# AdeeshKolluru/AdsorbDiff

Hardware: AMD Instinct MI355X
Metric: sampled adsorbate sites/sec (50 denoise steps, ~200-atom slabs) (higher is better)
Workload: dtype f32 (f16x3-split MFMA, fp32 accumulate; ADF_GEMM=f32 selects exact f32)

## Files before the change

adsorbdiff_amd/csrc/api.hip:

```cpp
#include <stdarg.h>
#include <stdlib.h>
#include <string.h>

#include <new>

#include "common.h"

static thread_local char g_err[512] = "";

void adf_set_error(const char* fmt, ...) {
    va_list ap;
    va_start(ap, fmt);
    vsnprintf(g_err, sizeof(g_err), fmt, ap);
    va_end(ap);
}

extern "C" const char* adf_last_error(void) { return g_err; }
extern "C" const char* adf_version(void) { return "adsorbdiff_hip 0.5.0 (gfx950)"; }

adf_tune adf_tune_from_env() {
    auto off_is_0 = [](const char* name) { const char* e = getenv(name); return (e && atoi(e) == 0) ? 0 : 1; };
    auto is_f32 = [](const char* name) { const char* e = getenv(name); return e && strcmp(e, "f32") == 0; };
    adf_tune t = {};
    t.gemm_stream = off_is_0("ADF_GEMM_STREAM");
    t.head_gate_fused = off_is_0("ADF_HEAD_GATE_FUSED");
    t.lift_emit = off_is_0("ADF_LIFT_EMIT");
    t.graph_sys_csr = off_is_0("ADF_GRAPH_SYS_CSR");
    t.train_gemm16 = is_f32("ADF_TRAIN_GEMM") ? 0 : 1;
    t.wgrad_f32 = is_f32("ADF_WGRAD") ? 1 : 0;
    const char* gt = getenv("ADF_EQV2_GEMM_TILE");
    t.eqv2_gemm_tile256 = (gt && atoi(gt) == 128) ? 0 : 1;
    t.eqv2_rotin_generic = getenv("ADF_EQV2_ROTIN_GENERIC") != nullptr;
    t.eqv2_rotout_generic = getenv("ADF_EQV2_ROTOUT_GENERIC") != nullptr;
    return t;
}
const adf_tune& adf_tune_process() {
    static const adf_tune t = adf_tune_from_env();
    return t;
}
int adf_current_num_cus() {
    int dev = 0, n = 0;
    if (hipGetDevice(&dev) != hipSuccess || hipDeviceGetAttribute(&n, hipDeviceAttributeMultiprocessorCount, dev) != hipSuccess) return 0;
    return n;
}

extern "C" int32_t adf_profile_enable(adf_painn_t h, int32_t on) {
    if (!h) { adf_set_error("null handle"); return ADF_EINVAL; }
    h->prof.enable(on != 0);
    ADF_HIP_CHECK(hipMemset(h->kcount, 0, 8 * sizeof(unsigned long long)));
    return ADF_OK;
}

extern "C" int32_t adf_profile_read(adf_painn_t h, float* ms, int64_t* count, int64_t* message_ksteps, void* stream) {
    if (!h || !ms || !count) { adf_set_error("null argument"); return ADF_EINVAL; }
    ADF_HIP_CHECK(hipStreamSynchronize((hipStream_t)stream));
    if (message_ksteps) {
        unsigned long long k[8];
        ADF_HIP_CHECK(hipMemcpy(k, h->kcount, sizeof(k), hipMemcpyDeviceToHost));
        ADF_HIP_CHECK(hipMemset(h->kcount, 0, sizeof(k)));
        *message_ksteps = (int64_t)k[0];
    }
    return h->prof.read(ms, count, ADF_PROF_NCAT);
// ... 347 lines not shown
    ADF_HIP_CHECK(hipMemcpyAsync(&e, h->nptr + N, sizeof(int32_t), hipMemcpyDeviceToHost, s));
    ADF_HIP_CHECK(hipStreamSynchronize(s));
    if (num_edges) *num_edges = e;
    return ADF_OK;
}

static int32_t zero_pad_rows(adf_painn* h, int N, hipStream_t s) {
    const size_t row = (size_t)5 * h->hp.hidden_channels;
    ADF_HIP_CHECK(hipMemsetAsync(h->rec + (size_t)N * row, 0, sizeof(float) * row, s));
    return ADF_OK;
}

static int32_t make_records(adf_painn* h, int l, int n, const float* x, const float* vec, bool vec_is_zero, float* rec,
                            const int32_t* row_map, hipStream_t s) {
    const int H = h->hp.hidden_channels;
    const adf_layer_weights& w = h->layer[l];
    if (n <= 0) return ADF_OK;
    adf_prof_begin(h, ADF_PROF_NODE, s);
    const bool lift = h->lift_on && !h->gemm_f32;
    const bool em = lift && h->tune.lift_emit;
    ADF_TRY(adf_nodewise_layernorm(x, w.ln_w, w.ln_b, h->y, n, H, s, em ? h->mag_a : nullptr, h->rows_dev));
    ADF_TRY(adf_linear(h, h->y, H, w.xp0_w, &w.xp0_16, w.xp0_b, h->cat, H, n, H, H, 1, s, em ? h->mag_a : nullptr,
                       em ? h->mag_b : nullptr));
    if (h->gemm_f32) {
        if (row_map) { adf_set_error("internal: mapped records need the f16x3 path"); return ADF_EINVAL; }
        ADF_TRY(adf_launch_gemm(h->cat, H, w.xp2_w, H, w.xp2_b, h->xh, 3 * H, n, 3 * H, H, 0, s));
        ADF_TRY(adf_pack_records(h, n, h->xh, vec, vec_is_zero, s, rec));
    } else {
        adf_epi ep = {};
        ep.vec_in = vec; ep.rec = rec ? rec : h->rec; ep.H = H; ep.vec_is_zero = vec_is_zero ? 1 : 0;
        ep.row_map = row_map;
        ep.rmag = em ? h->mag_b : nullptr;
        ep.m_dev = h->rows_dev;
        ADF_TRY(adf_launch_gemm16_fused(h->cat, H, &w.xp2_16, n, H, H, 1, &ep, s, h->tune, lift ? &h->lift : nullptr));
    }
    adf_prof_end(h, s);
    return ADF_OK;
}

static int32_t message_layer(adf_painn* h, int l, int N, const float* x, const float* vec, float* x_out,
                             float* vec_out, bool vec_is_zero, hipStream_t s, const int32_t* tlist = nullptr,
                             int n_targets = 0, float* rec = nullptr, bool records_ready = false) {
    if (!records_ready) ADF_TRY(make_records(h, l, N, x, vec, vec_is_zero, rec, nullptr, s));
    adf_prof_begin(h, ADF_PROF_MESSAGE, s);
    const int items = tlist ? n_targets : N;
    const bool emit = h->rmx && h->lift_on && !h->gemm_f32 && !h->msg_f32 && items > 0 && items <= h->part_stride;
    h->part_x = h->part_vec = nullptr;
    const int32_t st = adf_message_impl(h, l, N, x, h->xh, vec, x_out, vec_out, vec_is_zero, s, tlist, n_targets, rec,
                                        tlist ? h->rows_dev : nullptr, emit ? h->xpart : nullptr, h->vpart, h->part_stride);
    if (st == ADF_OK && emit) {
        h->part_x = x_out; h->part_vec = vec_out; h->part_n = items; h->part_dev = tlist ? h->rows_dev : nullptr;
        h->dbg_msg_rows = items;
    }
    adf_prof_end(h, s);
    return st;
}

static int32_t update_layer(adf_painn* h, int l, int N, float* x, float* vec, hipStream_t s, bool from_message = true) {
    const int H = h->hp.hidden_channels;
    const adf_layer_weights& w = h->layer[l];
    adf_prof_begin(h, ADF_PROF_NODE, s);
    const bool parts = from_message && h->rmx && h->lift_on && !h->gemm_f32 && N > 0 && h->part_x == x && h->part_vec == vec &&
                       h->part_n == N && h->part_dev == h->rows_dev;
    h->part_x = h->part_vec = nullptr;
    if (h->gemm_f32) {
        ADF_TRY(adf_launch_gemm(vec, H, w.vp_w, H, nullptr, h->vv, 2 * H, 3 * N, 2 * H, H, 0, s));
        ADF_TRY(adf_nodewise_update_prep(h->vv, x, h->cat, h->dot, N, H, s));
// ... 3 lines not shown
        ep.v1 = h->vv; ep.dotw = h->dot; ep.cat = h->cat; ep.H = H; ep.m_dev = h->rows_dev;
        const adf_lift* lf = h->lift_on ? &h->lift : nullptr;
        if (parts) {
            ADF_TRY(adf_launch_rowmax_combine(h->vpart, 3 * h->part_stride, H / ADF_SLICE_CH, 3ll * N, h->lift.buf, s, h->rows_dev, 3));
            ep.rmag = h->lift.buf;
            if (h->dbg_capture) ADF_HIP_CHECK(hipMemcpyAsync(h->dbg_mag, h->lift.buf, sizeof(float) * 3 * (size_t)N, hipMemcpyDeviceToDevice, s));
        }
        if (parts || (h->dbg_capture && h->rmx && lf && N <= h->part_stride)) {
            ep.catpart = h->catpart; ep.part_stride = h->part_stride; h->dbg_cat_rows = N;
        }
        ADF_TRY(adf_launch_gemm16_fused(vec, H, &w.vp_16, N, H, H, 3, &ep, s, h->tune, lf));
        if (parts) {
            ADF_TRY(adf_launch_rowmax_combine(h->xpart, h->part_stride, H / ADF_SLICE_CH + H / 32, N, h->lift.buf, s, h->rows_dev, 1));
            if (h->dbg_capture) {
                ADF_HIP_CHECK(hipMemcpyAsync(h->dbg_mag + 3 * h->part_stride, h->lift.buf, sizeof(float) * (size_t)N, hipMemcpyDeviceToDevice, s));
                h->dbg_comb_rows = N;
            }
        }
        adf_epi e0 = {};
        e0.A2 = h->cat; e0.K1 = H; e0.m_dev = h->rows_dev;
        e0.rmag = parts ? h->lift.buf : nullptr;
        e0.out_mag = h->lift_on ? reinterpret_cast<unsigned int*>(h->mag_b) : nullptr;
        ADF_TRY(adf_launch_gemm16(x, H, &w.xv0_16, w.xv0_b, h->y, H, N, H, 2 * H, 1, &e0, s, lf, h->tune, h->num_cus));
    }
    int32_t st;
    if (h->gemm_f32) {
        ADF_TRY(adf_launch_gemm(h->y, H, w.xv2_w, H, w.xv2_b, h->xh, 3 * H, N, 3 * H, H, 0, s));
        st = adf_nodewise_update_apply(h->xh, h->dot, h->vv, x, vec, h->scale[l], N, H, s);
    } else {
        adf_epi ep = {};
        ep.x = x; ep.vec = vec; ep.dot = h->dot; ep.vv = h->vv; ep.scale = h->scale[l]; ep.H = H;
        ep.rmag = h->lift_on ? h->mag_b : nullptr;
        ep.m_dev = h->rows_dev;
        st = adf_launch_gemm16_fused(h->y, H, &w.xv2_16, N, H, H, 2, &ep, s, h->tune);
    }
    adf_prof_end(h, s);
    return st;
}

extern "C" int32_t adf_painn_message_layer(adf_painn_t h, int32_t layer, int32_t N, const float* x, const float* vec,
                                           float* x_out, float* vec_out, void* stream) {
    if (!h || !h->weights_set || layer < 0 || layer >= h->hp.num_layers || N != h->lastN) {
        adf_set_error("message_layer: bad handle/layer, or N differs from the built graph");
        return ADF_EINVAL;
    }
    hipStream_t s = (hipStream_t)stream;
    ADF_TRY(zero_pad_rows(h, N, s));
    ADF_TRY(message_layer(h, layer, N, x, vec, x_out, vec_out, false, s));
    return ADF_OK;
}

extern "C" int32_t adf_painn_update_layer(adf_painn_t h, int32_t layer, int32_t N, float* x, float* vec, void* stream) {
    if (!h || !h->weights_set || layer < 0 || layer >= h->hp.num_layers) {
        adf_set_error("update_layer: bad handle/layer");
        return ADF_EINVAL;
    }
    ADF_TRY(ensure_capacity(h, N, 1));
    return update_layer(h, layer, N, x, vec, (hipStream_t)stream, false);
}

extern "C" int32_t adf_painn_get_tune(adf_painn_t h, adf_tune* out) {
    if (!h || !out) { adf_set_error("get_tune: null handle or output"); return ADF_EINVAL; }
    *out = h->tune;
    return ADF_OK;
}

extern "C" int32_t adf_painn_debug_row_maxima(adf_painn_t h, int32_t which, float* out, int64_t capacity, int32_t* rows,
// ... 527 lines not shown
```

adsorbdiff_amd/csrc/common.h:

```cpp
#pragma once
#include <hip/hip_runtime.h>
#include <stdint.h>
#include <stdio.h>
#include <string>
#include <vector>

#include "../../include/adsorbdiff_hip.h"

#define ADF_GROUP_NODES 32
#define ADF_SLICE_CH 64
#define ADF_MAX_CAND 1024
#define ADF_MAX_K 128
#define ADF_NFLAGS 8
#define ADF_MAX_INDEG 1024
#define ADF_MAX_LAYERS 16

void adf_set_error(const char* fmt, ...);

#define ADF_HIP_CHECK(expr)                                                             \
    do {                                                                                \
        hipError_t _e = (expr);                                                         \
        if (_e != hipSuccess) {                                                         \
            adf_set_error("%s failed: %s (%s:%d)", #expr, hipGetErrorString(_e),        \
                          __FILE__, __LINE__);                                          \
// ... 243 lines not shown
    int32_t last_reps[3];
    int num_cus;
    adf_prof prof;
    unsigned long long* kcount;
    adf_pool m_life;
    adf_pool m_ws;
    adf_pool m_inc;
    adf_pool m_sub;
    adf_pool m_rec0;
};

enum { ADF_PROF_GRAPH = 0, ADF_PROF_MESSAGE = 1, ADF_PROF_NODE = 2, ADF_PROF_HEADS = 3, ADF_PROF_STEPPER = 4 };
static inline void adf_prof_begin(adf_painn* h, int cat, hipStream_t s) { h->prof.begin(cat, s); }
static inline void adf_prof_end(adf_painn* h, hipStream_t s) { h->prof.end(s); }

int32_t adf_launch_gemm(const float* A, int lda, const float* W, int ldw, const float* bias, float* C, int ldc,
                        int M, int N, int K, int act_ssilu, hipStream_t s);
adf_tune adf_tune_from_env();
const adf_tune& adf_tune_process();
int adf_current_num_cus();
int32_t adf_launch_gemm16(const float* A, int lda, const adf_w16* W, const float* bias, float* C, int ldc, int M,
                          int N, int K, int act_ssilu, const adf_epi* ep, hipStream_t s, const adf_lift* lf,
                          const adf_tune& tune, int num_cus);
int32_t adf_launch_rowmag(const float* A, int lda, int K1, const float* A2, int K2, long long M, float* mag, hipStream_t s,
                          const int32_t* m_dev = nullptr, int m_mul = 1);
int32_t adf_launch_rowmax_combine(const float* part, long long stride, int nparts, long long M, float* mag, hipStream_t s,
                                  const int32_t* m_dev = nullptr, int m_mul = 1);
int32_t adf_split_weight(const float* w, long long n, adf_w16* out, unsigned int* scratch_bits, hipStream_t s,
                         int perm_H = 0, int K = 0, const float* bias = nullptr, int parts = 3);
int32_t adf_launch_gemm16_vecnorm(const float* A, int lda, const adf_w16* W, float* nrm, int M, int N, int K,
                                  hipStream_t s, const adf_tune& tune, const adf_lift* lf = nullptr,
                                  const float* premag = nullptr);
int32_t adf_launch_gemm16_fused(const float* A, int lda, const adf_w16* W, int M, int H, int K, int epi,
                                const adf_epi* ep, hipStream_t s, const adf_tune& tune, const adf_lift* lf = nullptr);
static inline int32_t adf_linear(const adf_painn* h, const float* A, int lda, const float* W, const adf_w16* W16,
                                 const float* bias, float* C, int ldc, int M, int N, int K, int act, hipStream_t s,
                                 const float* premag = nullptr, float* out_mag = nullptr) {
    if (h->gemm_f32) return adf_launch_gemm(A, lda, W, K, bias, C, ldc, M, N, K, act, s);
    adf_epi ep = {};
    ep.m_dev = h->rows_dev;
    if (h->lift_on) { ep.rmag = premag; ep.out_mag = reinterpret_cast<unsigned int*>(out_mag); }
    return adf_launch_gemm16(A, lda, W16, bias, C, ldc, M, N, K, act, &ep, s, h->lift_on ? &h->lift : nullptr, h->tune,
                             h->num_cus);
}
int32_t adf_pack_frag(const adf_w16* w, int N, int K, void* out, hipStream_t s);
int32_t adf_graph_build_impl(adf_painn* h, const adf_batch* b, hipStream_t s);
int32_t adf_energy_sum(const float* y, int H2, const float* w, const float* bias, const int32_t* atom_offset, float* energy,
                       int num_systems, hipStream_t s);
__device__ __forceinline__ float adf_row16_max(float v) {
#define ADF_ROR(n_) __int_as_float(__builtin_amdgcn_update_dpp(0, __float_as_int(v), 0x120 + (n_), 0xf, 0xf, false))
    v = fmaxf(v, ADF_ROR(8));
    v = fmaxf(v, ADF_ROR(4));
    v = fmaxf(v, ADF_ROR(2));
    v = fmaxf(v, ADF_ROR(1));
#undef ADF_ROR
    return v;
}
__device__ __forceinline__ float adf_half32_max_hi(float v) {
    v = adf_row16_max(v);
    return fmaxf(v, __int_as_float(__builtin_amdgcn_update_dpp(0, __float_as_int(v), 0x142, 0xa, 0xf, false)));
}
__device__ __forceinline__ float adf_lane8_max(float v) {
#define ADF_DPP(c_) __int_as_float(__builtin_amdgcn_update_dpp(0, __float_as_int(v), (c_), 0xf, 0xf, false))
    v = fmaxf(v, ADF_DPP(0xb1));
    v = fmaxf(v, ADF_DPP(0x4e));
    v = fmaxf(v, ADF_DPP(0x141));
#undef ADF_DPP
// ... 77 lines not shown
```

adsorbdiff_amd/csrc/gemm16.hip:

```cpp
#include <stdlib.h>

#include "common.h"

typedef float f32x16 __attribute__((ext_vector_type(16)));
typedef _Float16 half8 __attribute__((ext_vector_type(8)));
typedef _Float16 half4 __attribute__((ext_vector_type(4)));

#ifndef EPI_ABL
#define EPI_ABL 0
#endif
#ifndef G16_ABL
#define G16_ABL 0
#endif
#define HK 32
#define TLD3 96
#define TLD2 64
#define HLD 40

__device__ __forceinline__ float adf_pow2_lift(float mx) {
    if (!(mx > 0.f) || !(mx < 3.0e38f)) return 1.0f;
    int e;
    (void)frexpf(mx, &e);
    e = 15 - e;
    e = e > 120 ? 120 : (e < -120 ? -120 : e);
    return ldexpf(1.0f, e);
}

__device__ __forceinline__ float ssilu16(float x) {
    float s = x / (1.0f + expf(-x));
    return s * 1.6666666666666667f;
}

struct g16_tile {
    int NWN;
    int MI, NJ;
    int NT;
    int TM, TN;
    int ROWS;
};
constexpr g16_tile g16_tile_of(int epi, bool stream) {
    const int nwm = stream ? 1 : 2, nwn = stream ? 4 : 2;
    const int mi = epi >= 3 ? 3 : (epi ? 2 : (stream ? 3 : 2));
    const int nj = epi >= 3 ? 2 : (epi ? 3 : (stream ? 2 : 4));
    const int tm = 32 * mi * nwm;
    return {nwn, mi, nj, 64 * nwm * nwn, tm, 32 * nj * nwn, epi >= 3 ? tm / 3 : tm};
}

template <int ACT, int EPI, bool STREAM>
__global__ __launch_bounds__(g16_tile_of(EPI, STREAM).NT, 2) void adf_gemm_f16x3_kernel(
    const float* __restrict__ A, int lda, const _Float16* __restrict__ Whi, const _Float16* __restrict__ Wlo,
    const float* __restrict__ inv_scale, const float* __restrict__ bias, float* __restrict__ C, int ldc, int Mh, int N,
    int K, int tiles_n, adf_epi ep) {
    constexpr g16_tile geo = g16_tile_of(EPI, STREAM);
    constexpr int MI = geo.MI, NJ = geo.NJ, NWN = geo.NWN, NT = geo.NT, TM = geo.TM, TN = geo.TN;
    const int M = ep.m_dev ? min(Mh, (int)*ep.m_dev) : Mh;
    constexpr int NA = TM * 8 / NT;
    static_assert(TM * 8 % NT == 0, "A staging: whole float4s per thread");
    constexpr int LDS_STREAM = 4 * TM * HLD > NT / 64 * 6400 ? 4 * TM * HLD : NT / 64 * 6400;
    constexpr int LDS_MAIN = STREAM ? LDS_STREAM : (2 * TM + 2 * TN) * HLD;
    constexpr int LDS_REC = EPI == 1 ? NT / 64 * 2048 : 0;
    __shared__ __attribute__((aligned(16))) _Float16 lds[LDS_MAIN + LDS_REC];
    __shared__ float rinv[TM];
    _Float16* Ahi = lds;
    _Float16* Alo = Ahi + TM * HLD;
    _Float16* Bhi = Alo + TM * HLD;
    _Float16* Blo = Bhi + TN * HLD;
    const int tid = threadIdx.x;
    const int lane = tid & 63;
    const int wave = tid >> 6;
    const int wm = (wave / NWN) * (32 * MI);
    const int wn = (wave % NWN) * (32 * NJ);

    const int id = blockIdx.x;
    const int xcd = id & 7;
    const int qd = id >> 3;
    const int tile_m = (qd / tiles_n) * 8 + xcd;
    const int tile_n = qd % tiles_n;
    const int m0 = tile_m * geo.ROWS;
    const int n0 = tile_n * TN;
    if (m0 >= M) return;

    unsigned int a_goff[NA];
    int a_off[NA];
    float a_rs[NA];
    auto global_row = [&](int row) -> unsigned int {
        if constexpr (EPI >= 3) {
            const int atom = m0 + (row / 96) * 32 + (row & 31), ax = (row % 96) >> 5;
            return (unsigned int)min(atom, M - 1) * 3u + ax;
        } else {
            return (unsigned int)min(m0 + row, M - 1);
        }
    };
#pragma unroll
    for (int i = 0; i < NA; ++i) {
        const int f = tid + NT * i;
        const int row = f >> 3, kq = f & 7;
        const unsigned int grow = global_row(row);
        a_goff[i] = (grow * (unsigned int)lda + kq * 4) * 4u;
        a_off[i] = row * HLD + kq * 4;
        a_rs[i] = ep.rmag ? adf_pow2_lift(ep.rmag[grow]) : 1.0f;
    }
    if (tid < TM) rinv[tid] = ep.rmag ? 1.0f / adf_pow2_lift(ep.rmag[global_row(tid)]) : 1.0f;
    const char* const A1b = reinterpret_cast<const char*>(A);
    const char* const A2b = reinterpret_cast<const char*>(ep.A2) - (size_t)ep.K1 * 4;
    int w_src[NJ];
    int w_off[NJ];
#pragma unroll
    for (int i = 0; i < NJ; ++i) {
        const int f = tid + 256 * i;
        const int row = f >> 2, part = f & 3;
        w_src[i] = min(n0 + row, N - 1) * K + part * 8;
        w_off[i] = row * HLD + part * 8;
    }
// ... 310 lines not shown
            }
            if (ep.catpart) {
                const float mg = adf_lane8_max(fmaxf(fmaxf(fmaxf(0.f, fabsf(nv_.x)), fabsf(nv_.y)), fmaxf(fabsf(nv_.z), fabsf(nv_.w))));
                if (c4 == 0 && n < M) ep.catpart[(size_t)g * ep.part_stride + n] = mg;
            }
        }
    } else if constexpr (EPI == 4) {
        static_assert(EPI != 4 || (NJ == 2 && MI == 3), "norm epilogue: 3 components x 64 columns per wave");
        const int q = lane & 31;
        const int cb = n0 + wn;
        __syncthreads();
        float* T = reinterpret_cast<float*>(lds) + wave * 3200;
        const int a0 = m0 + (wave / NWN) * 32;
#pragma unroll
        for (int r = 0; r < 16; ++r) {
            const int lr = (r & 3) + 8 * (r >> 2) + 4 * (lane >> 5);
#pragma unroll
            for (int j = 0; j < 2; ++j) {
                const float a = acc[0][j][r] * (isc * rinv[wm + lr]), b = acc[1][j][r] * (isc * rinv[wm + 32 + lr]),
                            d = acc[2][j][r] * (isc * rinv[wm + 64 + lr]);
                T[lr * TLD2 + j * 32 + q] = sqrtf(a * a + b * b + d * d);
            }
        }
        __builtin_amdgcn_fence(__ATOMIC_RELEASE, "wavefront");
        __builtin_amdgcn_wave_barrier();
#pragma unroll
        for (int it = 0; it < 8; ++it) {
            const int lr = it * 4 + (lane >> 4), c4 = lane & 15;
            const int n = a0 + lr, c = cb + 4 * c4;
            if (n < M && c < N)
                *reinterpret_cast<float4*>(ep.cat + (size_t)n * N + c) = *reinterpret_cast<const float4*>(T + lr * TLD2 + 4 * c4);
        }
    } else {
        static_assert(EPI >= 3 || (NJ == 3 && MI == 2), "fused epilogues are written for the 64 x 96 wave tile");
        if (((EPI_ABL & 1) && EPI == 1) || ((EPI_ABL & 2) && EPI == 2)) {
            float sacc = 0.f;
            for (int i = 0; i < MI; ++i) for (int j = 0; j < NJ; ++j) for (int r = 0; r < 16; ++r) sacc += acc[i][j][r];
            if (ep.H < 0) ep.x[0] = sacc;
            return;
        }
        const int q = lane & 31;
        const int g = (n0 + wn) / 96;
        const int H = ep.H;
        const float b0 = bias[n0 + wn + q], b1 = bias[n0 + wn + 32 + q], b2 = bias[n0 + wn + 64 + q];
        __syncthreads();
        float* T = reinterpret_cast<float*>(lds) + wave * 3200;
#pragma unroll
        for (int i = 0; i < MI; ++i) {
#pragma unroll
            for (int r = 0; r < 16; ++r) {
                const int lr = (r & 3) + 8 * (r >> 2) + 4 * (lane >> 5);
                const float sc = isc * rinv[wm + 32 * i + lr];
                T[lr * TLD3 + q] = acc[i][0][r] * sc + b0;
                T[lr * TLD3 + 32 + q] = acc[i][1][r] * sc + b1;
                T[lr * TLD3 + 64 + q] = acc[i][2][r] * sc + b2;
            }
            __builtin_amdgcn_fence(__ATOMIC_RELEASE, "wavefront");
            __builtin_amdgcn_wave_barrier();
            const int c4 = lane & 7;
            const int c = 32 * g + 4 * c4;
            if constexpr (EPI == 1) {
                float4 v0[4], v1[4], v2[4];
                if (EPI_ABL & 4) { for (int it = 0; it < 4; ++it) { v0[it] = make_float4(1.f, 2.f, 3.f, 4.f); v1[it] = v0[it]; v2[it] = v0[it]; } }
                else if (!ep.vec_is_zero) {
#pragma unroll
                    for (int it = 0; it < 4; ++it) {
                        const int n = min(m0 + wm + 32 * i + it * 8 + (lane >> 3), M - 1);
// ... 55 lines not shown
                    }
                }
#pragma unroll
                for (int it = 0; it < 4; ++it) {
                    const int lr = it * 8 + (lane >> 3);
                    const int n = m0 + wm + 32 * i + lr;
                    const float4 p0 = *reinterpret_cast<const float4*>(T + lr * TLD3 + 4 * c4);
                    const float4 p1 = *reinterpret_cast<const float4*>(T + lr * TLD3 + 32 + 4 * c4);
                    const float4 p2 = *reinterpret_cast<const float4*>(T + lr * TLD3 + 64 + 4 * c4);
                    const float k2 = 0.70710678118654752f, sc = ep.scale;
                    float4 xo4 = xv[it];
                    xo4.x = (xo4.x + (p0.x + p1.x * d[it].x) * k2) * sc;
                    xo4.y = (xo4.y + (p0.y + p1.y * d[it].y) * k2) * sc;
                    xo4.z = (xo4.z + (p0.z + p1.z * d[it].z) * k2) * sc;
                    xo4.w = (xo4.w + (p0.w + p1.w * d[it].w) * k2) * sc;
                    if (n < M) {
                        *reinterpret_cast<float4*>(ep.x + (size_t)n * H + c) = xo4;
                        float* vr = ep.vec + (size_t)n * 3 * H + c;
#pragma unroll
                        for (int ax = 0; ax < 3; ++ax) {
                            float4 t = tv[it][ax];
                            const float4 v1 = w1[it][ax];
                            t.x += p2.x * v1.x; t.y += p2.y * v1.y; t.z += p2.z * v1.z; t.w += p2.w * v1.w;
                            *reinterpret_cast<float4*>(vr + ax * H) = t;
                        }
                    }
                }
            }
            __builtin_amdgcn_wave_barrier();
        }
    }
}

__global__ __launch_bounds__(256) void adf_rowmag_kernel(const float* __restrict__ A, int lda, int K1,
                                                         const float* __restrict__ A2, int K2, long long M,
                                                         float* __restrict__ mag, const int32_t* __restrict__ m_dev,
                                                         int m_mul) {
    const long long r = (long long)blockIdx.x * 4 + (threadIdx.x >> 6);
    const int lane = threadIdx.x & 63;
    if (r >= M || (m_dev && r >= (long long)*m_dev * m_mul)) return;
    float mx = 0.f;
    const float* a = A + (size_t)r * lda;
    for (int k = lane * 4; k < K1; k += 256) {
        const float4 v = *reinterpret_cast<const float4*>(a + k);
        mx = fmaxf(fmaxf(fmaxf(mx, fabsf(v.x)), fabsf(v.y)), fmaxf(fabsf(v.z), fabsf(v.w)));
    }
    if (A2) {
        const float* b = A2 + (size_t)r * lda;
        for (int k = lane * 4; k < K2; k += 256) {
            const float4 v = *reinterpret_cast<const float4*>(b + k);
            mx = fmaxf(fmaxf(fmaxf(mx, fabsf(v.x)), fabsf(v.y)), fmaxf(fabsf(v.z), fabsf(v.w)));
        }
    }
#pragma unroll
    for (int o = 32; o > 0; o >>= 1) mx = fmaxf(mx, __shfl_xor(mx, o));
    if (lane == 0) mag[r] = mx;
}

__global__ __launch_bounds__(256) void adf_rowmax_combine_kernel(const float* __restrict__ part, long long stride, int nparts,
                                                                 long long M, float* __restrict__ mag,
                                                                 const int32_t* __restrict__ m_dev, int m_mul) {
    const long long r = (long long)blockIdx.x * 256 + threadIdx.x;
    if (r >= M || (m_dev && r >= (long long)*m_dev * m_mul)) return;
    float mx = 0.f;
    for (int p = 0; p < nparts; ++p) mx = fmaxf(mx, part[(size_t)p * stride + r]);
    mag[r] = mx;
// ... 76 lines not shown
__global__ void adf_pack_frag_kernel(const _Float16* __restrict__ hi, const _Float16* __restrict__ lo, half8* __restrict__ out,
                                     int N, int K) {
    const int nks = K / 16;
    const long long total = (long long)(N / 32) * nks * 2 * 64;
    for (long long i = (long long)blockIdx.x * blockDim.x + threadIdx.x; i < total; i += (long long)gridDim.x * blockDim.x) {
        const int lane = (int)(i & 63), plane = (int)((i >> 6) & 1);
        const long long cs = i >> 7;
        const int s = (int)(cs % nks), cb = (int)(cs / nks);
        const _Float16* src = (plane ? lo : hi) + (size_t)(32 * cb + (lane & 31)) * K + 16 * s + 8 * (lane >> 5);
        out[i] = *reinterpret_cast<const half8*>(src);
    }
}

int32_t adf_pack_frag(const adf_w16* w, int N, int K, void* out, hipStream_t s) {
    if (N % 32 || K % 16) { adf_set_error("pack_frag: N %% 32 or K %% 16"); return ADF_EINVAL; }
    hipLaunchKernelGGL(adf_pack_frag_kernel, dim3(256), dim3(256), 0, s, (const _Float16*)w->hi, (const _Float16*)w->lo,
                       (half8*)out, N, K);
    ADF_HIP_CHECK(hipGetLastError());
    return ADF_OK;
}

static int32_t check_a_span(long long rows, int lda) {
    if (rows * (long long)lda * 4 >= (1ll << 32)) {
        adf_set_error("gemm16: A operand of %lld rows x %d exceeds the 32-bit offset range, split the batch", rows, lda);
        return ADF_EOOM;
    }
    return ADF_OK;
}

static bool can_stream(const adf_tune& tune, const adf_w16* W, int epi, int N, int K) {
    return tune.gemm_stream && W->frag && N % g16_tile_of(epi, true).TN == 0 && (K / HK) % 2 == 0;
}

static int32_t launch_f16x3(bool stream, int act, int epi, const float* A, int lda, const adf_w16* W, const float* bias, float* C,
                            int ldc, int M, int N, int K, const adf_epi& ep, hipStream_t s) {
    using kern_t = decltype(&adf_gemm_f16x3_kernel<0, 0, false>);
#define G16_FORM(STREAM_)                                                                                              \
    { adf_gemm_f16x3_kernel<0, 0, STREAM_>, adf_gemm_f16x3_kernel<1, 0, STREAM_>, adf_gemm_f16x3_kernel<0, 1, STREAM_>, \
      adf_gemm_f16x3_kernel<0, 2, STREAM_>, adf_gemm_f16x3_kernel<0, 3, STREAM_>, adf_gemm_f16x3_kernel<0, 4, STREAM_> }
    static const kern_t kernels[2][6] = {G16_FORM(false), G16_FORM(true)};
#undef G16_FORM
    const g16_tile t = g16_tile_of(epi, stream);
    const int tiles_n = (N + t.TN - 1) / t.TN;
    const int tiles_m8 = ((M + t.ROWS - 1) / t.ROWS + 7) / 8 * 8;
    hipLaunchKernelGGL(kernels[stream][epi ? epi + 1 : (act ? 1 : 0)], dim3((unsigned)(tiles_m8 * tiles_n)), dim3(t.NT), 0, s, A, lda,
                       (const _Float16*)(stream ? W->frag : W->hi), (const _Float16*)(stream ? nullptr : W->lo), W->inv_scale,
                       bias, C, ldc, M, N, K, tiles_n, ep);
    ADF_HIP_CHECK(hipGetLastError());
    return ADF_OK;
}

int32_t adf_launch_gemm16(const float* A, int lda, const adf_w16* W, const float* bias, float* C, int ldc, int M,
                          int N, int K, int act_ssilu, const adf_epi* ep_in, hipStream_t s, const adf_lift* lf,
                          const adf_tune& tune, int num_cus) {
    if (M <= 0) return ADF_OK;
    adf_epi ep = {};
    if (ep_in) ep = *ep_in;
    if (!ep.A2) ep.K1 = 0;
    if (K % HK != 0 || (lda & 3) || (ep.A2 && (ep.K1 <= 0 || ep.K1 % HK != 0 || ep.K1 >= K))) {
        adf_set_error("gemm16: K=%d (K1=%d) must be multiples of %d and lda a multiple of 4", K, ep.K1, HK);
        return ADF_EINVAL;
    }
    ADF_TRY(check_a_span(M, lda));
    if (ep.gate && (((N | ldc | ep.gate_ld) & 3) || (((uintptr_t)C | (uintptr_t)ep.gate) & 15))) {
        adf_set_error("gemm16: the gate epilogue needs N, ldc and gate_ld multiples of 4 and 16-byte aligned C and gate");
        return ADF_EINVAL;
    }
    ADF_TRY(lift_mags(A, lda, ep.A2 ? ep.K1 : K, ep.A2, ep.A2 ? K - ep.K1 : 0, M, lf, ep.rmag, &ep.rmag, s, ep.m_dev, 1));
    if (ep.out_mag) ADF_HIP_CHECK(hipMemsetAsync(ep.out_mag, 0, sizeof(float) * (size_t)M, s));
    const g16_tile ts = g16_tile_of(0, true);
    const long long wg = (long long)((M + ts.ROWS - 1) / ts.ROWS) * (N / ts.TN > 0 ? N / ts.TN : 1);
    const long long slots = 2ll * (num_cus > 0 ? num_cus : 256);
    const bool ragged4 = wg < 4 * slots && wg % slots != 0 && wg % slots < (3 * slots) / 10 && wg > slots;
    return launch_f16x3(can_stream(tune, W, 0, N, K) && !ragged4, act_ssilu, 0, A, lda, W, bias, C, ldc, M, N, K, ep, s);
}

int32_t adf_launch_gemm16_vecnorm(const float* A, int lda, const adf_w16* W, float* nrm, int M, int N, int K,
                                  hipStream_t s, const adf_tune& tune, const adf_lift* lf, const float* premag) {
    if (M <= 0) return ADF_OK;
    if (K % HK != 0 || (lda & 3) || (N & 3)) { adf_set_error("gemm16_vecnorm: bad shape"); return ADF_EINVAL; }
    ADF_TRY(check_a_span(3ll * M, lda));
    adf_epi ep = {};
    ep.cat = nrm;
    ADF_TRY(lift_mags(A, lda, K, nullptr, 0, 3ll * M, lf, premag, &ep.rmag, s));
    return launch_f16x3(can_stream(tune, W, 4, N, K), 0, 4, A, lda, W, nullptr, nullptr, 0, M, N, K, ep, s);
}

int32_t adf_launch_gemm16_fused(const float* A, int lda, const adf_w16* W, int M, int H, int K, int epi,
                                const adf_epi* ep_in, hipStream_t s, const adf_tune& tune, const adf_lift* lf) {
    adf_epi ep = *ep_in;
    if (M <= 0) return ADF_OK;
    if (K % HK != 0 || (lda & 3) || H % 64 != 0 || (epi != 3 && !W->bias_perm)) {
        adf_set_error("gemm16_fused: bad shape");
        return ADF_EINVAL;
    }
    const int rows_per = epi == 3 ? 3 : 1;
    ADF_TRY(check_a_span((long long)rows_per * M, lda));
    ADF_TRY(lift_mags(A, lda, K, nullptr, 0, (long long)rows_per * M, lf, ep_in->rmag, &ep.rmag, s, ep_in->m_dev, rows_per));
    const int N = (epi == 3 ? 2 : 3) * H;
    return launch_f16x3(can_stream(tune, W, epi, N, K), 0, epi, A, lda, W, epi == 3 ? nullptr : W->bias_perm, nullptr, 0, M, N, K, ep, s);
}
```

adsorbdiff_amd/lib.py:

```python
from __future__ import annotations

import ctypes as C
import re
from pathlib import Path

ADF_OK, ADF_EINVAL, ADF_EOOM, ADF_ENONEIGHBOR, ADF_EHIP, ADF_EOVERFLOW, ADF_ENUMERIC = 0, 1, 2, 3, 4, 5, 6


class NumericRangeError(ArithmeticError):
    """Non-finite model output (ADF_ENUMERIC).  Not a RuntimeError on purpose: ``ml_diffuse`` must not answer it by
    splitting the batch; the engine answers it by re-running in exact f32."""


class Hparams(C.Structure):
    _fields_ = [
        ("hidden_channels", C.c_int32), ("num_layers", C.c_int32), ("num_rbf", C.c_int32),
        ("num_elements", C.c_int32), ("max_neighbors", C.c_int32), ("envelope_exponent", C.c_int32),
        ("num_heads", C.c_int32), ("cutoff", C.c_float),
    ]


class EqV2Hparams(C.Structure):
    _fields_ = [
        ("lmax", C.c_int32), ("mmax", C.c_int32), ("num_layers", C.c_int32), ("sphere_channels", C.c_int32),
        ("attn_hidden_channels", C.c_int32), ("num_heads", C.c_int32), ("attn_alpha_channels", C.c_int32),
        ("attn_value_channels", C.c_int32), ("ffn_hidden_channels", C.c_int32), ("grid_resolution", C.c_int32),
        ("edge_channels", C.c_int32), ("num_distance_basis", C.c_int32), ("max_num_elements", C.c_int32),
        ("max_neighbors", C.c_int32), ("max_radius", C.c_float), ("avg_degree", C.c_float),
    ]


class EqV2Counters(C.Structure):
    _fields_ = [("num_edges", C.c_int64), ("num_atoms", C.c_int64), ("dense_flops", C.c_int64), ("conv_flops", C.c_int64),
                ("inc_rows", C.c_int64), ("inc_rows_full", C.c_int64), ("forwards_total", C.c_int64),
                ("conv_flops_total", C.c_int64)]


class Tune(C.Structure):
    _fields_ = [(name, C.c_int32) for name in (
        "gemm_stream", "head_gate_fused", "lift_emit", "graph_sys_csr", "train_gemm16", "wgrad_f32",
        "eqv2_gemm_tile256", "eqv2_rotin_generic", "eqv2_rotout_generic")]


class BatchDesc(C.Structure):
    _fields_ = [
        ("num_systems", C.c_int32), ("num_atoms", C.c_int32), ("pos", C.c_void_p), ("cell", C.c_void_p),
        ("atomic_numbers", C.c_void_p), ("batch", C.c_void_p), ("atom_offset", C.c_void_p), ("reps", C.c_int32 * 3),
    ]


class ActiveField(C.Structure):
    _fields_ = [("src", C.c_void_p), ("dst", C.c_void_p), ("row_bytes", C.c_int32), ("per_system", C.c_int32)]


class StepCoef(C.Structure):
    _fields_ = [
        ("coef_tr", C.c_float), ("rot_pre", C.c_float), ("rot_dt", C.c_float), ("rot_g2", C.c_float),
        ("noise_tr", C.c_float), ("noise_rot", C.c_float),
    ]


class TrCoef(C.Structure):
    _fields_ = [("coef", C.c_float), ("noise", C.c_float)]


class Counters(C.Structure):
    _fields_ = [
        ("num_edges", C.c_int64), ("num_atoms", C.c_int64), ("message_bytes_per_layer", C.c_int64),
        ("dense_flops", C.c_int64),
        ("inc_rows", C.c_int64), ("inc_rows_full", C.c_int64), ("inc_msg_launches", C.c_int64),
        ("inc_msg_edges", C.c_int64),
    ]


# ... 96 lines not shown
```

include/adsorbdiff_hip.h:

```cpp
#ifndef ADSORBDIFF_HIP_H
#define ADSORBDIFF_HIP_H

#include <stdint.h>

#ifdef __cplusplus
extern "C" {
#endif

#define ADF_OK 0
#define ADF_EINVAL 1
#define ADF_EOOM 2
#define ADF_ENONEIGHBOR 3
#define ADF_EHIP 4
#define ADF_EOVERFLOW 5
#define ADF_ENUMERIC 6

typedef struct adf_painn* adf_painn_t;

typedef struct {
    int32_t hidden_channels;
    int32_t num_layers;
    int32_t num_rbf;
    int32_t num_elements;
    int32_t max_neighbors;
// ... 7 lines not shown

int32_t adf_painn_create(const adf_painn_hparams* hp, adf_painn_t* out);
int32_t adf_painn_destroy(adf_painn_t h);

int32_t adf_painn_set_weights(adf_painn_t h, int32_t n_weights, const void* const* weights,
                              const float* scale_factors, void* stream);

typedef struct {
    int32_t num_systems;
    int32_t num_atoms;
    const float* pos;
    const float* cell;
    const int32_t* atomic_numbers;
    const int32_t* batch;
    const int32_t* atom_offset;
    int32_t reps[3];
} adf_batch;

int32_t adf_graph_build(adf_painn_t h, const adf_batch* b, void* stream, int64_t* num_edges);

int32_t adf_graph_set_moving(adf_painn_t h, const int32_t* moving, const int32_t* mov_idx, const int32_t* mov_off);

int32_t adf_painn_set_arithmetic(adf_painn_t h, int32_t exact_f32);

int32_t adf_painn_set_incremental(adf_painn_t h, int32_t on);

typedef struct adf_tune {
    int32_t gemm_stream;
    int32_t head_gate_fused;
    int32_t lift_emit;
    int32_t graph_sys_csr;
    int32_t train_gemm16;
    int32_t wgrad_f32;
    int32_t eqv2_gemm_tile256;
    int32_t eqv2_rotin_generic;
    int32_t eqv2_rotout_generic;
} adf_tune;
int32_t adf_painn_get_tune(adf_painn_t h, adf_tune* out);

int32_t adf_check_flags(adf_painn_t h, void* stream);

int32_t adf_graph_export(adf_painn_t h, int32_t* nbr_count, int32_t* nbr_src, int32_t* nbr_shift,
                         int64_t edge_capacity, int32_t* edge_src, int32_t* edge_dst, float* edge_dist,
                         float* edge_vec, int64_t* num_edges, void* stream);

int32_t adf_painn_forward(adf_painn_t h, const adf_batch* b, float* f1, float* f2, void* stream);

int32_t adf_painn_forward_subset(adf_painn_t h, const adf_batch* b, const int32_t* out_idx, int32_t n_out, float* f1,
                                 float* f2, void* stream);

int32_t adf_painn_message_layer(adf_painn_t h, int32_t layer, int32_t num_atoms, const float* x,
                                const float* vec, float* x_out, float* vec_out, void* stream);
int32_t adf_painn_update_layer(adf_painn_t h, int32_t layer, int32_t num_atoms, float* x, float* vec,
                               void* stream);
int32_t adf_painn_debug_row_maxima(adf_painn_t h, int32_t which, float* out, int64_t capacity, int32_t* rows,
                                   void* stream);

int32_t adf_linear_forward(const float* A, const float* W, const float* bias, float* C, int32_t M, int32_t N,
                           int32_t K, int32_t act_ssilu, int32_t mode, void* stream);

typedef struct {
    float coef_tr;
    float rot_pre;
    float rot_dt;
    float rot_g2;
    float noise_tr;
// ... 417 lines not shown
```

Baseline: 262.6.

## Add cost-model tile policy mixing short M-panels to fill GEMM wave tails

Moves the f16x3 GEMM body into a device function templated on the panel height, so a streamed launch can mix full-height and shorter (1 or 2 sub-block) row panels. A host-side cost model, using per-epilogue constants and the CU slot count, picks a panel mix that reduces the ragged last wave of workgroups. It also re-decides between the staged and streamed paths with that model. This adds kernel instantiations (code size and register pressure) and depends on hand-fit cost constants, with an env knob to turn it off.

```diff
diff --git a/adsorbdiff_amd/csrc/api.hip b/adsorbdiff_amd/csrc/api.hip
--- a/adsorbdiff_amd/csrc/api.hip
+++ b/adsorbdiff_amd/csrc/api.hip
@@ -28,6 +28,9 @@
     t.graph_sys_csr = off_is_0("ADF_GRAPH_SYS_CSR");
     t.train_gemm16 = is_f32("ADF_TRAIN_GEMM") ? 0 : 1;
     t.wgrad_f32 = is_f32("ADF_WGRAD") ? 1 : 0;
+    t.gemm_tile_policy = off_is_0("ADF_GEMM_TILE_POLICY");
+    const char* sl = getenv("ADF_GEMM_TILE_SLOTS");
+    t.gemm_tile_slots = (sl && atoi(sl) > 0) ? atoi(sl) : 0;
     const char* gt = getenv("ADF_EQV2_GEMM_TILE");
     t.eqv2_gemm_tile256 = (gt && atoi(gt) == 128) ? 0 : 1;
     t.eqv2_rotin_generic = getenv("ADF_EQV2_ROTIN_GENERIC") != nullptr;
@@ -441,7 +444,7 @@
         ep.row_map = row_map;
         ep.rmag = em ? h->mag_b : nullptr;
         ep.m_dev = h->rows_dev;
-        ADF_TRY(adf_launch_gemm16_fused(h->cat, H, &w.xp2_16, n, H, H, 1, &ep, s, h->tune, lift ? &h->lift : nullptr));
+        ADF_TRY(adf_launch_gemm16_fused(h->cat, H, &w.xp2_16, n, H, H, 1, &ep, s, h->tune, lift ? &h->lift : nullptr, h->num_cus));
     }
     adf_prof_end(h, s);
     return ADF_OK;
@@ -511,7 +514,7 @@
         ep.x = x; ep.vec = vec; ep.dot = h->dot; ep.vv = h->vv; ep.scale = h->scale[l]; ep.H = H;
         ep.rmag = h->lift_on ? h->mag_b : nullptr;
         ep.m_dev = h->rows_dev;
-        st = adf_launch_gemm16_fused(h->y, H, &w.xv2_16, N, H, H, 2, &ep, s, h->tune);
+        st = adf_launch_gemm16_fused(h->y, H, &w.xv2_16, N, H, H, 2, &ep, s, h->tune, nullptr, h->num_cus);
     }
     adf_prof_end(h, s);
     return st;
diff --git a/adsorbdiff_amd/csrc/common.h b/adsorbdiff_amd/csrc/common.h
--- a/adsorbdiff_amd/csrc/common.h
+++ b/adsorbdiff_amd/csrc/common.h
@@ -299,7 +299,8 @@
                                   hipStream_t s, const adf_tune& tune, const adf_lift* lf = nullptr,
                                   const float* premag = nullptr);
 int32_t adf_launch_gemm16_fused(const float* A, int lda, const adf_w16* W, int M, int H, int K, int epi,
-                                const adf_epi* ep, hipStream_t s, const adf_tune& tune, const adf_lift* lf = nullptr);
+                                const adf_epi* ep, hipStream_t s, const adf_tune& tune, const adf_lift* lf = nullptr,
+                                int num_cus = 0);
 static inline int32_t adf_linear(const adf_painn* h, const float* A, int lda, const float* W, const adf_w16* W16,
                                  const float* bias, float* C, int ldc, int M, int N, int K, int act, hipStream_t s,
                                  const float* premag = nullptr, float* out_mag = nullptr) {
diff --git a/adsorbdiff_amd/csrc/gemm16.hip b/adsorbdiff_amd/csrc/gemm16.hip
--- a/adsorbdiff_amd/csrc/gemm16.hip
+++ b/adsorbdiff_amd/csrc/gemm16.hip
@@ -1,6 +1,9 @@
 #include <stdlib.h>
 
+#include <atomic>
+
 #include "common.h"
+#include "tile_policy.h"
 
 typedef float f32x16 __attribute__((ext_vector_type(16)));
 typedef _Float16 half8 __attribute__((ext_vector_type(8)));
@@ -45,22 +48,24 @@
     const int tm = 32 * mi * nwm;
     return {nwn, mi, nj, 64 * nwm * nwn, tm, 32 * nj * nwn, epi >= 3 ? tm / 3 : tm};
 }
-
-template <int ACT, int EPI, bool STREAM>
-__global__ __launch_bounds__(g16_tile_of(EPI, STREAM).NT, 2) void adf_gemm_f16x3_kernel(
-    const float* __restrict__ A, int lda, const _Float16* __restrict__ Whi, const _Float16* __restrict__ Wlo,
-    const float* __restrict__ inv_scale, const float* __restrict__ bias, float* __restrict__ C, int ldc, int Mh, int N,
-    int K, int tiles_n, adf_epi ep) {
+constexpr int g16_lds_main(int epi, bool stream) {
+    const g16_tile t = g16_tile_of(epi, stream);
+    const int lds_stream = 4 * t.TM * HLD > t.NT / 64 * 6400 ? 4 * t.TM * HLD : t.NT / 64 * 6400;
+    return stream ? lds_stream : (2 * t.TM + 2 * t.TN) * HLD;
+}
+
+template <int ACT, int EPI, bool STREAM, int MI>
+__device__ __forceinline__ void g16_tile_body(_Float16* __restrict__ lds, float* __restrict__ rinv, const float* __restrict__ A, int lda,
+                                              const _Float16* __restrict__ Whi, const _Float16* __restrict__ Wlo,
+                                              const float* __restrict__ inv_scale, const float* __restrict__ bias,
+                                              float* __restrict__ C, int ldc, int M, int N, int K, int m0, int n0, const adf_epi& ep) {
     constexpr g16_tile geo = g16_tile_of(EPI, STREAM);
-    constexpr int MI = geo.MI, NJ = geo.NJ, NWN = geo.NWN, NT = geo.NT, TM = geo.TM, TN = geo.TN;
-    const int M = ep.m_dev ? min(Mh, (int)*ep.m_dev) : Mh;
+    constexpr int NJ = geo.NJ, NWN = geo.NWN, NT = geo.NT, TN = geo.TN;
+    constexpr int TM = 32 * MI * (4 / NWN);
+    static_assert(MI >= 1 && MI <= geo.MI && (MI == geo.MI || (STREAM && EPI < 3)), "short panels: streamed EPI 0 / 1 / 2 only");
     constexpr int NA = TM * 8 / NT;
     static_assert(TM * 8 % NT == 0, "A staging: whole float4s per thread");
-    constexpr int LDS_STREAM = 4 * TM * HLD > NT / 64 * 6400 ? 4 * TM * HLD : NT / 64 * 6400;
-    constexpr int LDS_MAIN = STREAM ? LDS_STREAM : (2 * TM + 2 * TN) * HLD;
-    constexpr int LDS_REC = EPI == 1 ? NT / 64 * 2048 : 0;
-    __shared__ __attribute__((aligned(16))) _Float16 lds[LDS_MAIN + LDS_REC];
-    __shared__ float rinv[TM];
+    constexpr int LDS_MAIN = g16_lds_main(EPI, STREAM);
     _Float16* Ahi = lds;
     _Float16* Alo = Ahi + TM * HLD;
     _Float16* Bhi = Alo + TM * HLD;
@@ -70,15 +75,6 @@
     const int wave = tid >> 6;
     const int wm = (wave / NWN) * (32 * MI);
     const int wn = (wave % NWN) * (32 * NJ);
-
-    const int id = blockIdx.x;
-    const int xcd = id & 7;
-    const int qd = id >> 3;
-    const int tile_m = (qd / tiles_n) * 8 + xcd;
-    const int tile_n = qd % tiles_n;
-    const int m0 = tile_m * geo.ROWS;
-    const int n0 = tile_n * TN;
-    if (m0 >= M) return;
 
     unsigned int a_goff[NA];
     int a_off[NA];
@@ -455,7 +451,7 @@
                 *reinterpret_cast<float4*>(ep.cat + (size_t)n * N + c) = *reinterpret_cast<const float4*>(T + lr * TLD2 + 4 * c4);
         }
     } else {
-        static_assert(EPI >= 3 || (NJ == 3 && MI == 2), "fused epilogues are written for the 64 x 96 wave tile");
+        static_assert(EPI >= 3 || (NJ == 3 && geo.MI == 2), "fused epilogues are written for the 64 x 96 wave tile");
         if (((EPI_ABL & 1) && EPI == 1) || ((EPI_ABL & 2) && EPI == 2)) {
             float sacc = 0.f;
             for (int i = 0; i < MI; ++i) for (int j = 0; j < NJ; ++j) for (int r = 0; r < 16; ++r) sacc += acc[i][j][r];
@@ -577,6 +573,38 @@
     }
 }
 
+template <int ACT, int EPI, bool STREAM>
+__global__ __launch_bounds__(g16_tile_of(EPI, STREAM).NT, 2) void adf_gemm_f16x3_kernel(
+    const float* __restrict__ A, int lda, const _Float16* __restrict__ Whi, const _Float16* __restrict__ Wlo,
+    const float* __restrict__ inv_scale, const float* __restrict__ bias, float* __restrict__ C, int ldc, int Mh, int N,
+    int K, int tiles_n, adf_epi ep, adf_tile_plan plan) {
+    constexpr g16_tile geo = g16_tile_of(EPI, STREAM);
+    const int M = ep.m_dev ? min(Mh, (int)*ep.m_dev) : Mh;
+    constexpr int LDS_REC = EPI == 1 ? geo.NT / 64 * 2048 : 0;
+    __shared__ __attribute__((aligned(16))) _Float16 lds[g16_lds_main(EPI, STREAM) + LDS_REC];
+    __shared__ float rinv[geo.TM];
+    int panel, tile_n;
+    adf_tile_map(blockIdx.x, tiles_n, panel, tile_n);
+    const int n0 = tile_n * geo.TN;
+#define G16_BODY(MI_) g16_tile_body<ACT, EPI, STREAM, MI_>(lds, rinv, A, lda, Whi, Wlo, inv_scale, bias, C, ldc, M, N, K, m0, n0, ep)
+    if constexpr (STREAM && EPI < 3) {
+        int block0, mi;
+        adf_tile_panel(plan.n, geo.MI, panel, block0, mi);
+        const int m0 = block0 * 32;
+        if (mi == 0 || m0 >= M) return;
+        if (mi == geo.MI) { G16_BODY(geo.MI); return; }
+        if constexpr (geo.MI == 3) {
+            if (mi == 2) { G16_BODY(2); return; }
+        }
+        G16_BODY(1);
+    } else {
+        const int m0 = panel * geo.ROWS;
+        if (m0 >= M) return;
+        G16_BODY(geo.MI);
+    }
+#undef G16_BODY
+}
+
 __global__ __launch_bounds__(256) void adf_rowmag_kernel(const float* __restrict__ A, int lda, int K1,
                                                          const float* __restrict__ A2, int K2, long long M,
                                                          float* __restrict__ mag, const int32_t* __restrict__ m_dev,
@@ -719,8 +747,49 @@
     return tune.gemm_stream && W->frag && N % g16_tile_of(epi, true).TN == 0 && (K / HK) % 2 == 0;
 }
 
+#define G16_C0_EPI0 10.0f
+#define G16_C1_EPI0 14.5f
+#define G16_C0_EPI1 12.8f
+#define G16_C1_EPI1 20.1f
+#define G16_C0_EPI2 13.4f
+#define G16_C1_EPI2 20.8f
+#define G16_T_STAGED 86.5f
+#define G16_POLICY_MAX_ROUNDS 16
+static adf_tile_cost g16_cost_of(int epi) {
+    switch (epi) {
+        case 0: return {G16_C0_EPI0, G16_C1_EPI0};
+        case 1: return {G16_C0_EPI1, G16_C1_EPI1};
+        default: return {G16_C0_EPI2, G16_C1_EPI2};
+    }
+}
+static int g16_slots(const adf_tune& tune, int num_cus) {
+    return tune.gemm_tile_slots > 0 ? tune.gemm_tile_slots : 2 * (num_cus > 0 ? num_cus : 256);
+}
+static std::atomic<long long> g16_mixed_launches{0};
+extern "C" int64_t adf_gemm16_mixed_launches(void) { return g16_mixed_launches.load(); }
+
+static adf_tile_plan g16_plan_of(const adf_tune& tune, bool stream, int epi, int M, int N, int num_cus) {
+    const g16_tile t = g16_tile_of(epi, stream);
+    if (!stream || epi >= 3) {
+        adf_tile_plan u = {};
+        u.n[0] = u.panels = (M + t.ROWS - 1) / t.ROWS;
+        return u;
+    }
+#ifdef G16_FORCE_MI
+    {
+        const int h = G16_FORCE_MI < t.MI ? G16_FORCE_MI : t.MI;
+        adf_tile_plan f = {};
+        f.n[t.MI - h] = f.panels = (int)(((M + 31) / 32 + h - 1) / h);
+        f.mixed = h != t.MI;
+        return f;
+    }
+#endif
+    if (!tune.gemm_tile_policy) return adf_tile_uniform(M, t.MI);
+    return adf_tile_policy(M, (N + t.TN - 1) / t.TN, g16_slots(tune, num_cus), t.MI, g16_cost_of(epi), G16_POLICY_MAX_ROUNDS);
+}
+
 static int32_t launch_f16x3(bool stream, int act, int epi, const float* A, int lda, const adf_w16* W, const float* bias, float* C,
-                            int ldc, int M, int N, int K, const adf_epi& ep, hipStream_t s) {
+                            int ldc, int M, int N, int K, const adf_epi& ep, hipStream_t s, const adf_tile_plan& plan) {
     using kern_t = decltype(&adf_gemm_f16x3_kernel<0, 0, false>);
 #define G16_FORM(STREAM_)                                                                                              \
     { adf_gemm_f16x3_kernel<0, 0, STREAM_>, adf_gemm_f16x3_kernel<1, 0, STREAM_>, adf_gemm_f16x3_kernel<0, 1, STREAM_>, \
@@ -729,10 +798,10 @@
 #undef G16_FORM
     const g16_tile t = g16_tile_of(epi, stream);
     const int tiles_n = (N + t.TN - 1) / t.TN;
-    const int tiles_m8 = ((M + t.ROWS - 1) / t.ROWS + 7) / 8 * 8;
-    hipLaunchKernelGGL(kernels[stream][epi ? epi + 1 : (act ? 1 : 0)], dim3((unsigned)(tiles_m8 * tiles_n)), dim3(t.NT), 0, s, A, lda,
-                       (const _Float16*)(stream ? W->frag : W->hi), (const _Float16*)(stream ? nullptr : W->lo), W->inv_scale,
-                       bias, C, ldc, M, N, K, tiles_n, ep);
+    if (plan.mixed) g16_mixed_launches.fetch_add(1, std::memory_order_relaxed);
+    hipLaunchKernelGGL(kernels[stream][epi ? epi + 1 : (act ? 1 : 0)], dim3((unsigned)adf_tile_grid(plan.panels, tiles_n)), dim3(t.NT), 0,
+                       s, A, lda, (const _Float16*)(stream ? W->frag : W->hi), (const _Float16*)(stream ? nullptr : W->lo),
+                       W->inv_scale, bias, C, ldc, M, N, K, tiles_n, ep, plan);
     ADF_HIP_CHECK(hipGetLastError());
     return ADF_OK;
 }
@@ -755,11 +824,22 @@
     }
     ADF_TRY(lift_mags(A, lda, ep.A2 ? ep.K1 : K, ep.A2, ep.A2 ? K - ep.K1 : 0, M, lf, ep.rmag, &ep.rmag, s, ep.m_dev, 1));
     if (ep.out_mag) ADF_HIP_CHECK(hipMemsetAsync(ep.out_mag, 0, sizeof(float) * (size_t)M, s));
-    const g16_tile ts = g16_tile_of(0, true);
+    const g16_tile ts = g16_tile_of(0, true), tl = g16_tile_of(0, false);
     const long long wg = (long long)((M + ts.ROWS - 1) / ts.ROWS) * (N / ts.TN > 0 ? N / ts.TN : 1);
     const long long slots = 2ll * (num_cus > 0 ? num_cus : 256);
-    const bool ragged4 = wg < 4 * slots && wg % slots != 0 && wg % slots < (3 * slots) / 10 && wg > slots;
-    return launch_f16x3(can_stream(tune, W, 0, N, K) && !ragged4, act_ssilu, 0, A, lda, W, bias, C, ldc, M, N, K, ep, s);
+    bool staged = wg < 4 * slots && wg % slots != 0 && wg % slots < (3 * slots) / 10 && wg > slots;
+#ifdef G16_FORCE_MI
+    staged = false;
+#endif
+    const bool stream = can_stream(tune, W, 0, N, K);
+    adf_tile_plan plan = g16_plan_of(tune, stream, 0, M, N, num_cus);
+    if (stream && staged && tune.gemm_tile_policy) {
+        const int ps = g16_slots(tune, num_cus);
+        const long long wgl = (long long)((M + tl.ROWS - 1) / tl.ROWS) * ((N + tl.TN - 1) / tl.TN);
+        staged = (double)((wgl + ps - 1) / ps) * G16_T_STAGED < adf_tile_model_time(plan.n, ts.MI, (N + ts.TN - 1) / ts.TN, ps, g16_cost_of(0));
+    }
+    if (stream && staged) plan = g16_plan_of(tune, false, 0, M, N, num_cus);
+    return launch_f16x3(stream && !staged, act_ssilu, 0, A, lda, W, bias, C, ldc, M, N, K, ep, s, plan);
 }
 
 int32_t adf_launch_gemm16_vecnorm(const float* A, int lda, const adf_w16* W, float* nrm, int M, int N, int K,
@@ -770,11 +850,12 @@
     adf_epi ep = {};
     ep.cat = nrm;
     ADF_TRY(lift_mags(A, lda, K, nullptr, 0, 3ll * M, lf, premag, &ep.rmag, s));
-    return launch_f16x3(can_stream(tune, W, 4, N, K), 0, 4, A, lda, W, nullptr, nullptr, 0, M, N, K, ep, s);
+    const bool stream = can_stream(tune, W, 4, N, K);
+    return launch_f16x3(stream, 0, 4, A, lda, W, nullptr, nullptr, 0, M, N, K, ep, s, g16_plan_of(tune, stream, 4, M, N, 0));
 }
 
 int32_t adf_launch_gemm16_fused(const float* A, int lda, const adf_w16* W, int M, int H, int K, int epi,
-                                const adf_epi* ep_in, hipStream_t s, const adf_tune& tune, const adf_lift* lf) {
+                                const adf_epi* ep_in, hipStream_t s, const adf_tune& tune, const adf_lift* lf, int num_cus) {
     adf_epi ep = *ep_in;
     if (M <= 0) return ADF_OK;
     if (K % HK != 0 || (lda & 3) || H % 64 != 0 || (epi != 3 && !W->bias_perm)) {
@@ -785,5 +866,7 @@
     ADF_TRY(check_a_span((long long)rows_per * M, lda));
     ADF_TRY(lift_mags(A, lda, K, nullptr, 0, (long long)rows_per * M, lf, ep_in->rmag, &ep.rmag, s, ep_in->m_dev, rows_per));
     const int N = (epi == 3 ? 2 : 3) * H;
-    return launch_f16x3(can_stream(tune, W, epi, N, K), 0, epi, A, lda, W, epi == 3 ? nullptr : W->bias_perm, nullptr, 0, M, N, K, ep, s);
-}
+    const bool stream = can_stream(tune, W, epi, N, K);
+    return launch_f16x3(stream, 0, epi, A, lda, W, epi == 3 ? nullptr : W->bias_perm, nullptr, 0, M, N, K, ep, s,
+                        g16_plan_of(tune, stream, epi, M, N, num_cus));
+}
diff --git a/adsorbdiff_amd/csrc/tile_policy.h b/adsorbdiff_amd/csrc/tile_policy.h
--- /dev/null
+++ b/adsorbdiff_amd/csrc/tile_policy.h
@@ -0,0 +1,90 @@
+#pragma once
+
+#define ADF_TILE_MAX_MI 3
+#define ADF_TILE_INLINE __attribute__((always_inline))
+
+struct adf_tile_cost {
+    float c0, c1;
+};
+
+struct adf_tile_plan {
+    int n[ADF_TILE_MAX_MI];
+    int panels;
+    int mixed;
+};
+
+ADF_TILE_INLINE constexpr void adf_tile_panel(const int (&n)[ADF_TILE_MAX_MI], int MI, int p, int& block0, int& mi) {
+    const int n0 = n[0], n1 = MI >= 2 ? n[1] : 0, n2 = MI >= 3 ? n[2] : 0;
+    if (p < n0) { block0 = p * MI; mi = MI; return; }
+    p -= n0;
+    int b = n0 * MI;
+    if (p < n1) { block0 = b + p * (MI - 1); mi = MI - 1; return; }
+    p -= n1;
+    b += n1 * (MI - 1);
+    if (p < n2) { block0 = b + p * (MI - 2); mi = MI - 2; return; }
+    block0 = b + n2 * (MI - 2);
+    mi = 0;
+}
+
+constexpr int adf_tile_grid(int panels, int tiles_n) { return (panels + 7) / 8 * 8 * tiles_n; }
+ADF_TILE_INLINE constexpr void adf_tile_map(int id, int tiles_n, int& panel, int& tile_n) {
+    const int qd = id >> 3;
+    panel = (qd / tiles_n) * 8 + (id & 7);
+    tile_n = qd % tiles_n;
+}
+
+inline double adf_tile_model_time(const int (&n)[ADF_TILE_MAX_MI], int MI, int tiles_n, int slots, adf_tile_cost c) {
+    long long pos = 0;
+    double t = 0.0;
+    for (int k = 0; k < MI; ++k) {
+        const long long cnt = (long long)n[k] * tiles_n;
+        if (cnt == 0) continue;
+        const long long first = (pos + slots - 1) / slots, end = (pos + cnt + slots - 1) / slots;
+        if (end > first) t += (double)(end - first) * ((double)c.c0 + (double)c.c1 * (MI - k));
+        pos += cnt;
+    }
+    return t;
+}
+
+inline adf_tile_plan adf_tile_uniform(long long rows, int MI) {
+    adf_tile_plan u = {};
+    const long long blocks = (rows + 31) / 32;
+    u.n[0] = (int)((blocks + MI - 1) / MI);
+    u.panels = u.n[0];
+    return u;
+}
+
+inline adf_tile_plan adf_tile_policy(long long rows, int tiles_n, int slots, int MI, adf_tile_cost c, int max_rounds) {
+    adf_tile_plan best = adf_tile_uniform(rows, MI);
+    if (MI <= 1 || MI > ADF_TILE_MAX_MI || rows <= 0 || tiles_n <= 0 || slots <= 0 || !(c.c1 > 0.f) || c.c0 < 0.f) return best;
+    const long long blocks = (rows + 31) / 32;
+    double best_t = adf_tile_model_time(best.n, MI, tiles_n, slots, c);
+    const double eps = 1e-9 * best_t;
+    const long long rounds_u = ((long long)best.n[0] * tiles_n + slots - 1) / slots;
+    if (max_rounds > 0 && rounds_u > max_rounds) return best;
+    long long tall_prev = -1;
+    for (int back = 0; back <= 3; ++back) {
+        long long tall = blocks / MI;
+        if (back > 0) {
+            const long long r = rounds_u - back;
+            if (r < 0) break;
+            const long long fit = r * slots / tiles_n;
+            if (fit < tall) tall = fit;
+        }
+        if (tall == tall_prev) continue;
+        tall_prev = tall;
+        const long long rest = blocks - tall * MI;
+        if (rest == 0) continue;
+        for (int h = MI - 1; h >= 1; --h) {
+            adf_tile_plan p = {};
+            p.n[0] = (int)tall;
+            p.n[MI - h] += (int)(rest / h);
+            if (rest % h) p.n[MI - (int)(rest % h)] += 1;
+            for (int k = 0; k < MI; ++k) p.panels += p.n[k];
+            p.mixed = 1;
+            const double t = adf_tile_model_time(p.n, MI, tiles_n, slots, c);
+            if (t < best_t - eps) { best = p; best_t = t; }
+        }
+    }
+    return best;
+}
diff --git a/adsorbdiff_amd/lib.py b/adsorbdiff_amd/lib.py
--- a/adsorbdiff_amd/lib.py
+++ b/adsorbdiff_amd/lib.py
@@ -39,7 +39,7 @@
 class Tune(C.Structure):
     _fields_ = [(name, C.c_int32) for name in (
         "gemm_stream", "head_gate_fused", "lift_emit", "graph_sys_csr", "train_gemm16", "wgrad_f32",
-        "eqv2_gemm_tile256", "eqv2_rotin_generic", "eqv2_rotout_generic")]
+        "gemm_tile_policy", "gemm_tile_slots", "eqv2_gemm_tile256", "eqv2_rotin_generic", "eqv2_rotout_generic")]
 
 
 class BatchDesc(C.Structure):
diff --git a/include/adsorbdiff_hip.h b/include/adsorbdiff_hip.h
--- a/include/adsorbdiff_hip.h
+++ b/include/adsorbdiff_hip.h
@@ -63,6 +63,8 @@
     int32_t graph_sys_csr;
     int32_t train_gemm16;
     int32_t wgrad_f32;
+    int32_t gemm_tile_policy;
+    int32_t gemm_tile_slots;
     int32_t eqv2_gemm_tile256;
     int32_t eqv2_rotin_generic;
     int32_t eqv2_rotout_generic;
```

Result: no change. 263.0 (median of 6 runs) (+0.2%).
